# DuckTapeDevOps/kubernetes-cloud

Measured on AMD Instinct MI355X. Metric: GPT-J-6B finetune tokens/sec, higher is better.
Workload: dtype bf16; 1 GPU; model=gpt-j-6b, global_batch=32, micro_batch=16, grad_accum=2, seq_len=2048, parallelism=dp1, activation_checkpointing=False

## Files before the change

csrc/kernels/attention.hip:

```cpp
#include "common.h"

#define LOG2E 1.4426950408889634f
#define LN2 0.6931471805599453f

struct AttnParams {
  const bf16_t* q; const bf16_t* k; const bf16_t* v;
  bf16_t* o; float* lse;
  long long q_sb, q_st, q_sh, k_sb, k_st, k_sh, v_sb, v_st, v_sh;
  long long o_sb, o_st, o_sh;
  int B, Sq, Sk, H, Hkv, d_real, causal;
  float scale;
  const float* alibi;
  const int* kv_len;
  const int* fix_flags;
  int window;
  const unsigned* key_mask;
  int km_words;
};

struct AttnBwdParams {
  const bf16_t* q; const bf16_t* k; const bf16_t* v; const bf16_t* o;
  const bf16_t* dout; bf16_t* dq; bf16_t* dk; bf16_t* dv;
  const float* lse; const float* delta;
  long long q_sb, q_st, q_sh, k_sb, k_st, k_sh, v_sb, v_st, v_sh;
// ... 886 lines not shown
    if (causal) {
      hipLaunchKernelGGL((attn_bwd_dkdv_kernel<256, true>), g1w, dim3(256), 0, stream, p);
      hipLaunchKernelGGL((attn_bwd_dq32_kernel<256, true>), h2, dim3(256), 0, stream, p);
    } else {
      hipLaunchKernelGGL((attn_bwd_dkdv_kernel<256, false>), g1w, dim3(256), 0, stream, p);
      hipLaunchKernelGGL((attn_bwd_dq32_kernel<256, false>), h2, dim3(256), 0, stream, p);
    }
    return 0;
  }
  dim3 g1(((Sk + 63) / 64) * B * Hkv);
  dim3 g2(((Sq + 63) / 64) * B * H);
  ATTN_D_DISPATCH(D, {
    if (causal) {
      hipLaunchKernelGGL((attn_bwd_dkdv_kernel<DD, true>), g1, dim3(256), 0, stream, p);
      hipLaunchKernelGGL((attn_bwd_dq_kernel<DD, true>), g2, dim3(256), 0, stream, p);
    } else {
      hipLaunchKernelGGL((attn_bwd_dkdv_kernel<DD, false>), g1, dim3(256), 0, stream, p);
      hipLaunchKernelGGL((attn_bwd_dq_kernel<DD, false>), g2, dim3(256), 0, stream, p);
    }
  });
  return 0;
}

KCA_API int kca_attn_bwd(const void* q, const void* k, const void* v,
                         const void* o, const void* dout, void* dq, void* dk,
                         void* dv, const float* lse, const float* delta,
                         long long q_sb, long long q_st, long long q_sh,
                         long long k_sb, long long k_st, long long k_sh,
                         long long v_sb, long long v_st, long long v_sh,
                         long long do_sb, long long do_st, long long do_sh,
                         long long dq_sb, long long dq_st, long long dq_sh,
                         long long dk_sb, long long dk_st, long long dk_sh,
                         long long dv_sb, long long dv_st, long long dv_sh,
                         int B, int Sq, int Sk, int H, int Hkv, int d_real,
                         int causal, float scale, const float* alibi,
                         const int* kv_len, int window, const unsigned* key_mask, hipStream_t stream) {
  return kca_attn_bwd_ws(q, k, v, o, dout, dq, dk, dv, lse, delta, q_sb, q_st, q_sh, k_sb, k_st, k_sh, v_sb, v_st,
                         v_sh, do_sb, do_st, do_sh, dq_sb, dq_st, dq_sh, dk_sb, dk_st, dk_sh, dv_sb, dv_st, dv_sh,
                         B, Sq, Sk, H, Hkv, d_real, causal, scale, alibi, kv_len, window, key_mask, nullptr, 0,
                         stream);
}
```

csrc/kernels/attention_tiled.hip:

```cpp
#include "common.h"

#include <type_traits>

namespace {

constexpr float kLog2e = 1.4426950408889634f;
constexpr float kLn2 = 0.6931471805599453f;
constexpr float kRescaleThr = 8.0f;

#ifdef KCA_ATTN_STAMPS
__device__ unsigned long long g_attn_stamps[64];
__device__ __forceinline__ unsigned long long ast_now() {
  unsigned long long t;
  __builtin_amdgcn_sched_barrier(0);
  asm volatile("s_memtime %0\n\ts_waitcnt lgkmcnt(0)" : "=s"(t)::"memory");
  __builtin_amdgcn_sched_barrier(0);
  return t;
}
#define ASTAMP_DECL                                            \
  unsigned long long st_acc_[8] = {0, 0, 0, 0, 0, 0, 0, 0}; \
  unsigned long long st_prev_ = ast_now();
#define ASTAMP(k)                           \
  do {                                      \
    const unsigned long long n_ = ast_now(); \
// ... 206 lines not shown
  constexpr int NCH = D / 8, RB = D * 2, NCS = DS / 8;
  const int l32 = lane & 31, hh = lane >> 5;
#pragma unroll
  for (int db = 0; db < D / 32; ++db) {
#pragma unroll
    for (int g = 0; g < 4; ++g) {
      uint2 w;
      w.x = pk_bf16(acc[db][4 * g] * mul, acc[db][4 * g + 1] * mul);
      w.y = pk_bf16(acc[db][4 * g + 2] * mul, acc[db][4 * g + 3] * mul);
      *reinterpret_cast<uint2*>(lds + l32 * RB + ((4 * db + g + l32) % NCH) * 16 + hh * 8) = w;
    }
  }
  asm volatile("" ::: "memory");
  static_assert((32 * NCS) % 64 == 0, "whole-wave epilogue rounds");
#pragma unroll
  for (int j = 0; j < 32 * NCS / 64; ++j) {
    const int idx = j * 64 + lane, r = idx / NCS, c = idx % NCS;
    const uint4 v = *reinterpret_cast<const uint4*>(lds + r * RB + ((c + r) % NCH) * 16);
    *reinterpret_cast<uint4*>(row0 + (long long)r * st + c * 8) = v;
  }
  asm volatile("" ::: "memory");
}

template <int D, bool CAUSAL, int OC = -1, int DS = D, int MC = -1>
__global__ void __launch_bounds__(256, (D <= 128 ? 2 : 1)) attn_fwd_tiled_kernel(FastFwdParams p) {
  constexpr int BM = 128, BN = 32;
  constexpr int TILE = BN * D * 2;
  constexpr int KS = DS / 16;
  using Stg = StagerFor<D, DS>;
  constexpr int CPT = Stg::CPT;
  __shared__ __attribute__((aligned(16))) char smem[3 * 2 * TILE];

  ASTAMP_DECL
  const int tid = threadIdx.x, lane = tid & 63, wave = tid >> 6;
  const int l32 = lane & 31, hh = lane >> 5, gi = lane & 15;
  const int nqb = p.Sq / BM;
  const int lid = xcd_remap(blockIdx.x, gridDim.x);
  const int qi = lid % nqb;
  const int qb = CAUSAL ? (nqb - 1 - qi) : qi;
  const int bh = lid / nqb;
  const int b = bh / p.H, h = bh % p.H;
  const int hk = h / (p.H / p.Hkv);
  const int off = p.Sk - p.Sq;
  const int q0 = qb * BM + wave * 32;
  const int qrow = q0 + l32;
  int kv_hi = p.Sk;
// ... 420 lines not shown
  const float inv = ltot > 0.f ? 1.f / ltot : 0.f;
  if (hh == 0 && p.lse)
    p.lse[((long long)b * p.H + h) * p.Sq + qrow] = ltot > 0.f ? (m + log2f(ltot)) * kLn2 : INFINITY;
  asm volatile("s_waitcnt vmcnt(0) lgkmcnt(0)" ::: "memory");
  __syncthreads();
  store_tile_lds<D, D>(p.o + b * p.o_sb + h * p.o_sh + (long long)q0 * p.o_st, p.o_st, oacc, lane, inv,
                       smem + wave * 32 * D * 2);
  ASTAMP(6);
  ASTAMP_FLUSH(48);
}

struct FastBwdParams {
  const bf16_t* q; const bf16_t* k; const bf16_t* v; const bf16_t* dout;
  bf16_t* dq; bf16_t* dk; bf16_t* dv;
  const float* lse; const float* delta;
  long long q_sb, q_st, q_sh, k_sb, k_st, k_sh, v_sb, v_st, v_sh, do_sb, do_st, do_sh;
  long long dq_sb, dq_st, dq_sh, dk_sb, dk_st, dk_sh, dv_sb, dv_st, dv_sh;
  int B, Sq, Sk, H, Hkv;
  float scale;
};
struct FastBwdWsParams : FastBwdParams {
  bf16_t* ws;
};

template <int D>
__device__ __forceinline__ void row_bases(int l32, int hh, int& e, int& o) {
  const int xr = (l32 >> 2) & 3;
  e = (l32 >> 3) * 16 * D + 64 * (l32 & 7) + 16 * (hh ^ xr);
  o = (l32 >> 3) * 16 * D + 64 * (l32 & 7) + 16 * ((2 + hh) ^ xr);
}
template <int D>
__device__ __forceinline__ void tr_bases(int lane, int& b1, int& b2) {
  const int hh = lane >> 5, gi = lane & 15;
  const int c3 = 2 * ((lane >> 4) & 1) + ((gi & 3) >> 1);
  b1 = 64 * (4 * hh + (gi >> 2)) + 16 * (c3 ^ hh) + 8 * (gi & 1);
  b2 = 16 * D + 64 * (4 * hh + (gi >> 2)) + 16 * (c3 ^ hh ^ 2) + 8 * (gi & 1);
}
template <int D>
__device__ __forceinline__ bf16x8 tr_frag(const char* img, int b1, int b2, int s, int db) {
  return cat8(lds_tr4(img, b1 + 2 * s * 16 * D + 512 * db), lds_tr4(img, b2 + 2 * s * 16 * D + 512 * db));
}
template <int D>
__device__ __forceinline__ bf16x8 row_frag(const char* img, int be, int bo, int s) {
  return lds_b128(img, ((s & 1) ? bo : be) + 512 * (s >> 1));
}

// ... 132 lines not shown
          t1[(db + 1) & 1] = tr_frag<D>(Ks, b1, b2, 1, db + 1);
          __builtin_amdgcn_sched_group_barrier(0x100, 4, 0);
        }
        dq[db] = __builtin_amdgcn_mfma_f32_32x32x16_bf16(t0[db & 1], d0, dq[db], 0, 0, 0);
        dq[db] = __builtin_amdgcn_mfma_f32_32x32x16_bf16(t1[db & 1], d1, dq[db], 0, 0, 0);
        __builtin_amdgcn_sched_group_barrier(0x8, 2, 0);
      }
    }
    ASTAMP(4);
    asm volatile("" ::: "memory");
    if (t + 1 < ntiles) stg.store(sk, sv, smem + ((t + 1) & 1) * 2 * TILE);
    __syncthreads();
    ASTAMP(5);
  };
  const int nfree = CAUSAL ? ntiles - 4 : ntiles;
  for (int t = 0; t < nfree; ++t) tile_step(t, std::false_type{});
  for (int t = max(nfree, 0); t < ntiles; ++t) tile_step(t, std::true_type{});
  store_tile_lds<D, DS>(p.dq + b * p.dq_sb + h * p.dq_sh + (long long)q0 * p.dq_st, p.dq_st, dq, lane, p.scale,
                        smem + wave * 32 * D * 2);
  ASTAMP(6);
  ASTAMP_FLUSH(16);
}

template <int D, bool CAUSAL>
__global__ void __launch_bounds__(256, 2) attn_bwd_dq_ds_kernel(FastBwdWsParams p) {
  constexpr int BM = 128, BN = 32;
  constexpr int TILE = BN * D * 2;
  constexpr int NCH = D / 8, CPT = 32 * NCH / 256, RPI = 256 / NCH;
  constexpr int DST = BN * 32 * 2;
  constexpr int DOFF = 2 * TILE;
  __shared__ __attribute__((aligned(16))) char smem[4 * TILE];
  static_assert(DOFF + 2 * 4 * DST <= 4 * TILE && 256 % NCH == 0, "dQ from dS: LDS plan");

  const int tid = threadIdx.x, lane = tid & 63, wave = tid >> 6;
  const int hh = lane >> 5;
  const int nqb = p.Sq / BM;
  const int lid = xcd_remap(blockIdx.x, gridDim.x);
  const int qi = lid % nqb;
  const int qb = CAUSAL ? (nqb - 1 - qi) : qi;
  const int bh = lid / nqb;
  const int b = bh / p.H, h = bh % p.H;
  const int off = p.Sk - p.Sq;
  const int q0 = qb * BM + wave * 32;
  int kv_hi = p.Sk;
  if (CAUSAL) kv_hi = min(kv_hi, qb * BM + BM + off);
  const int ntiles = (kv_hi + BN - 1) / BN;

  f32x16 dq[D / 32];
// ... 73 lines not shown
      t0[0] = tr_frag<D>(Ks, b1, b2, 0, 0);
      t1[0] = tr_frag<D>(Ks, b1, b2, 1, 0);
      __builtin_amdgcn_sched_group_barrier(0x100, 8, 0);
#pragma unroll
      for (int db = 0; db < D / 32; ++db) {
        if (db + 1 < D / 32) {
          t0[(db + 1) & 1] = tr_frag<D>(Ks, b1, b2, 0, db + 1);
          t1[(db + 1) & 1] = tr_frag<D>(Ks, b1, b2, 1, db + 1);
          __builtin_amdgcn_sched_group_barrier(0x100, 4, 0);
        }
        dq[db] = __builtin_amdgcn_mfma_f32_32x32x16_bf16(t0[db & 1], d0, dq[db], 0, 0, 0);
        dq[db] = __builtin_amdgcn_mfma_f32_32x32x16_bf16(t1[db & 1], d1, dq[db], 0, 0, 0);
        __builtin_amdgcn_sched_group_barrier(0x8, 2, 0);
      }
    }
    asm volatile("" ::: "memory");
    if (t + 1 < ntiles) store_tile((t + 1) & 1, std::integral_constant<int, NX>{});
    load_k(min(t + 2, last));
    load_ds(min(t + 1 + PD, last), std::integral_constant<int, NX>{});
    __syncthreads();
  };
  for (int t = 0; t < ntiles; t += PD)
    static_for<0, PD>([&](auto J) { tile_step(t + decltype(J)::value, J); });
  store_tile_lds<D>(p.dq + b * p.dq_sb + h * p.dq_sh + (long long)q0 * p.dq_st, p.dq_st, dq, lane, p.scale,
                    smem + wave * 32 * D * 2);
}

template <int D, bool CAUSAL, int DS = D>
__global__ void __launch_bounds__(256, (D <= 64 && !CAUSAL) ? 3 : 1) attn_bwd_dkdv_tiled_kernel(FastBwdParams p) {
  constexpr int BK = 128, BQ = 32;
  constexpr int TILE = BQ * D * 2;
  using Stg = StagerFor<D, DS>;
  constexpr int NCH = D / 8, NCS = DS / 8, CPT = Stg::CPT;
  constexpr int KSD = DS / 16;
  constexpr int VOFF = 4 * TILE;
  constexpr int LOFF = VOFF + 4 * TILE;
  __shared__ __attribute__((aligned(16))) char smem[LOFF + 2 * 64 * 4];
  ASTAMP_DECL

  const int tid = threadIdx.x, lane = tid & 63, wave = tid >> 6;
  const int l32 = lane & 31, hh = lane >> 5;
  const int nkb = p.Sk / BK;
  const int lid = xcd_remap(blockIdx.x, gridDim.x);
  const int kb = lid % nkb, bh = lid / nkb;
  const int b = bh / p.Hkv, hk = bh % p.Hkv;
  const int grp = p.H / p.Hkv;
  const int off = p.Sk - p.Sq;
  const int kw = kb * BK + wave * 32;
// ... 171 lines not shown

template <bool ON>
struct DsEmitter {
  __device__ __forceinline__ void init(const FastBwdParams&, int, int, int, int) {}
  __device__ __forceinline__ void store(const bf16x8&, const bf16x8&, int) const {}
};
template <>
struct DsEmitter<true> {
  __amdgpu_buffer_rsrc_t r_;
  int v_, dt_, t0_;
  __device__ __forceinline__ void init(const FastBwdWsParams& p, int bh, int lane, int q_lo, int kw) {
    r_ = head_rsrc(p.ws + (long long)bh * p.Sq * p.Sk);
    v_ = lane * 16;
    dt_ = (p.Sk / 32) * 2048;
    t0_ = (q_lo / 32) * dt_ + (kw / 32) * 2048;
  }
  __device__ __forceinline__ void store(const bf16x8& s0, const bf16x8& s1, int t) const {
    const int so = __builtin_amdgcn_readfirstlane(t0_ + t * dt_);
    __builtin_amdgcn_raw_buffer_store_b128(*reinterpret_cast<const u32x4*>(&s0), r_, v_, so, 2);
    __builtin_amdgcn_raw_buffer_store_b128(*reinterpret_cast<const u32x4*>(&s1), r_, v_, so + 1024, 2);
  }
};

template <int D, bool CAUSAL, bool EMIT_DS = false>
__global__ void __launch_bounds__(512, 1)
    attn_bwd_dkdv_w8_kernel(std::conditional_t<EMIT_DS, FastBwdWsParams, FastBwdParams> p) {
  constexpr int BK = 128, BQ = 32;
  constexpr int TILE = BQ * D * 2;
  using Stg = Stager<D, true, 512>;
  constexpr int CPT = Stg::CPT, KSD = D / 16;
  constexpr int PSZ = 4 * 64 * 16;
  constexpr int POFF = 3 * 2 * TILE;
  constexpr int LOFF = POFF + 2 * 4 * PSZ;
  __shared__ __attribute__((aligned(16))) char smem[LOFF + 3 * 64 * 4];
  static_assert(8 * 32 * D * 2 <= LOFF, "epilogue images of the 8 waves");
  ASTAMP_DECL

  const int tid = threadIdx.x, lane = tid & 63;
  const int wave = __builtin_amdgcn_readfirstlane(tid >> 6);
  const int pw = wave & 3;
  const bool kside = wave < 4;
  const int l32 = lane & 31, hh = lane >> 5;
  const int nkb = p.Sk / BK;
  const int lid = xcd_remap(blockIdx.x, gridDim.x);
  const int kb = lid % nkb, bh = lid / nkb;
  const int b = bh / p.H, h = bh % p.H;
  const int off = p.Sk - p.Sq;
  const int kw = kb * BK + pw * 32;
  const int key = kw + l32;
// ... 187 lines not shown
      }
      ASTAMP(4);
      asm volatile("" ::: "memory");
      if (t + 2 < total) store_tile(nxt);
      __syncthreads();
      ASTAMP(5);
    };
    if (total > 1) {
      load_tile(1);
      store_tile(1);
    }
    __syncthreads();
    int cur = 0;
    for (int t = 0; t < total; ++t) {
      const int nxt = cur == 0 ? 2 : cur - 1;
      k_step(t, cur, nxt);
      cur = cur == 2 ? 0 : cur + 1;
    }
  }
  __builtin_amdgcn_s_setprio(0);
  {
    bf16_t* dst = kside ? p.dk + b * p.dk_sb + h * p.dk_sh + (long long)kw * p.dk_st
                        : p.dv + b * p.dv_sb + h * p.dv_sh + (long long)kw * p.dv_st;
    store_tile_lds<D>(dst, kside ? p.dk_st : p.dv_st, acc, lane, kside ? p.scale : 1.f, smem + wave * 32 * D * 2);
  }
  ASTAMP(6);
  if (!kside) {
    ASTAMP_FLUSH(40);
  } else {
    ASTAMP_FLUSH(56);
  }
}

inline bool offsets_fit(long long rows, long long stride) { return (rows + 128) * stride * 2 < (1ll << 31); }

}

static int g_attn_variant = 7;
KCA_API int kca_attn_set_variant(int v) {
  g_attn_variant = v;
  return 0;
}

KCA_API int kca_attn_fwd_tiled(const void* q, const void* k, const void* v, void* o, float* lse,
                               long long q_sb, long long q_st, long long q_sh, long long k_sb,
                               long long k_st, long long k_sh, long long v_sb, long long v_st,
                               long long v_sh, long long o_sb, long long o_st, long long o_sh,
                               int B, int Sq, int Sk, int H, int Hkv, int d, int causal,
                               float scale, int rowsum_col, int max_col, int* flags, hipStream_t stream) {
  if ((d != 48 && d != 64 && d != 96 && d != 128 && d != 160 && d != 256) || Sq % 128 || Sk % 32 || Sq <= 0 ||
      H % Hkv || !flags)
    return 1;
  if (max_col >= 0 && (max_col != 40 || rowsum_col != 40 || d != 48)) return 1;
  if (d == 48 && causal) return 1;
  if (rowsum_col >= 0 && (rowsum_col != 40 || (d != 64 && d != 48) || causal)) return 1;
  if (causal && Sk < Sq) return 1;
  if (!offsets_fit(Sk, k_st) || !offsets_fit(Sk, v_st)) return 1;
  FastFwdParams p{(const bf16_t*)q, (const bf16_t*)k, (const bf16_t*)v, (bf16_t*)o, lse, flags,
                  q_sb, q_st, q_sh, k_sb, k_st, k_sh, v_sb, v_st, v_sh, o_sb, o_st, o_sh,
                  B, Sq, Sk, H, Hkv, scale};
  dim3 grid((Sq / 128) * B * H);
// ... 131 lines not shown
  const long long need = kca_attn_bwd_ws_bytes(B, Sq, Sk, H, Hkv, d, causal);
  if ((g_attn_variant & 6) != 6 || !ws || need == 0 || ws_bytes < need || !offsets_fit(Sk, k_st) ||
      !offsets_fit(Sk, v_st) || !offsets_fit(Sq, q_st) || !offsets_fit(Sq, do_st))
    return kca_attn_bwd_tiled(q, k, v, dout, dq, dk, dv, lse, delta, q_sb, q_st, q_sh, k_sb, k_st, k_sh, v_sb,
                              v_st, v_sh, do_sb, do_st, do_sh, dq_sb, dq_st, dq_sh, dk_sb, dk_st, dk_sh, dv_sb,
                              dv_st, dv_sh, B, Sq, Sk, H, Hkv, d, causal, scale, stream);
  FastBwdWsParams p{{(const bf16_t*)q, (const bf16_t*)k, (const bf16_t*)v, (const bf16_t*)dout,
                     (bf16_t*)dq, (bf16_t*)dk, (bf16_t*)dv, lse, delta,
                     q_sb, q_st, q_sh, k_sb, k_st, k_sh, v_sb, v_st, v_sh, do_sb, do_st, do_sh,
                     dq_sb, dq_st, dq_sh, dk_sb, dk_st, dk_sh, dv_sb, dv_st, dv_sh,
                     B, Sq, Sk, H, Hkv, scale},
                    (bf16_t*)ws};
  dim3 g1((Sk / 128) * B * H), g2((Sq / 128) * B * H);
  if (causal) {
    hipLaunchKernelGGL((attn_bwd_dkdv_w8_kernel<256, true, true>), g1, dim3(512), 0, stream, p);
    hipLaunchKernelGGL((attn_bwd_dq_ds_kernel<256, true>), g2, dim3(256), 0, stream, p);
  } else {
    hipLaunchKernelGGL((attn_bwd_dkdv_w8_kernel<256, false, true>), g1, dim3(512), 0, stream, p);
    hipLaunchKernelGGL((attn_bwd_dq_ds_kernel<256, false>), g2, dim3(256), 0, stream, p);
  }
  return 0;
}

#ifdef KCA_ATTN_STAMPS
KCA_API int kca_attn_stamps(unsigned long long* host, int reset) {
  if (hipMemcpyFromSymbol(host, HIP_SYMBOL(g_attn_stamps), sizeof(unsigned long long) * 64) != hipSuccess) return 1;
  if (reset) {
    unsigned long long z[64] = {0};
    if (hipMemcpyToSymbol(HIP_SYMBOL(g_attn_stamps), z, sizeof(z)) != hipSuccess) return 1;
  }
  return 0;
}
#endif
```

csrc/kernels/common.h:

```cpp
#pragma once
#include <hip/hip_runtime.h>
#include <hip/hip_bf16.h>
#include <stdint.h>

#define KCA_API extern "C" __attribute__((visibility("default")))

typedef uint16_t bf16_t;
typedef float f32x4 __attribute__((ext_vector_type(4)));
typedef float f32x16 __attribute__((ext_vector_type(16)));
typedef short s16x8 __attribute__((ext_vector_type(8)));
typedef short s16x4 __attribute__((ext_vector_type(4)));
typedef __bf16 bf16x8 __attribute__((ext_vector_type(8)));
typedef __bf16 bf16x4 __attribute__((ext_vector_type(4)));

#ifdef KCA_DEBUG
#define KCA_DASSERT(cond)                                                                                  \
  do {                                                                                                     \
    if (!(cond)) {                                                                                         \
      printf("KCA_DASSERT failed %s:%d: %s (block %d,%d,%d thread %d)\n", __FILE__, __LINE__, #cond,         \
             (int)blockIdx.x, (int)blockIdx.y, (int)blockIdx.z, (int)threadIdx.x);                         \
      __builtin_trap();                                                                                    \
    }                                                                                                      \
  } while (0)
#else
// ... 7 lines not shown
  return __uint_as_float(((uint32_t)b) << 16);
}

__device__ __forceinline__ uint16_t f2bf(float f) {
  __bf16 h = (__bf16)f;
  return __builtin_bit_cast(uint16_t, h);
}

__device__ __forceinline__ uint32_t pack_bf16x2(float lo, float hi) {
  return (uint32_t)f2bf(lo) | ((uint32_t)f2bf(hi) << 16);
}

__device__ __forceinline__ void load8(const bf16_t* p, float (&x)[8]) {
  U16x8 u = *reinterpret_cast<const U16x8*>(p);
#pragma unroll
  for (int i = 0; i < 8; ++i) x[i] = bf2f(u.v[i]);
}

__device__ __forceinline__ void store8(bf16_t* p, const float (&x)[8]) {
  U16x8 u;
#pragma unroll
  for (int i = 0; i < 8; ++i) u.v[i] = f2bf(x[i]);
  *reinterpret_cast<U16x8*>(p) = u;
}

__device__ __forceinline__ void load8f(const float* p, float (&x)[8]) {
  float4 a = *reinterpret_cast<const float4*>(p);
  float4 b = *reinterpret_cast<const float4*>(p + 4);
  x[0] = a.x; x[1] = a.y; x[2] = a.z; x[3] = a.w;
  x[4] = b.x; x[5] = b.y; x[6] = b.z; x[7] = b.w;
}

__device__ __forceinline__ void store8f(float* p, const float (&x)[8]) {
  *reinterpret_cast<float4*>(p) = make_float4(x[0], x[1], x[2], x[3]);
  *reinterpret_cast<float4*>(p + 4) = make_float4(x[4], x[5], x[6], x[7]);
}

template <int DT>
__device__ __forceinline__ float e2f(uint32_t u16) {
  if constexpr (DT == 0) return __uint_as_float(u16 << 16);
  else return (float)__builtin_bit_cast(_Float16, (uint16_t)u16);
}
template <int DT>
__device__ __forceinline__ uint32_t f2e(float f) {
  if constexpr (DT == 0) return (uint32_t)f2bf(f);
  else return (uint32_t)__builtin_bit_cast(uint16_t, (_Float16)f);
// ... 110 lines not shown
```

csrc/kernels/elementwise.hip:

```cpp
#include "common.h"

__device__ __forceinline__ float gelu_erf(float x) {
  return 0.5f * x * (1.f + erff(x * 0.7071067811865476f));
}
__device__ __forceinline__ float gelu_erf_grad(float x) {
  const float cdf = 0.5f * (1.f + erff(x * 0.7071067811865476f));
  const float pdf = 0.3989422804014327f * __expf(-0.5f * x * x);
  return cdf + x * pdf;
}

template <bool TANH, int DT = 0>
__global__ void gelu_fwd_kernel(const bf16_t* __restrict__ u,
                                bf16_t* __restrict__ y, long long n8) {
  for (long long i = blockIdx.x * (long long)blockDim.x + threadIdx.x; i < n8;
       i += (long long)gridDim.x * blockDim.x) {
    float v[8];
    load8_t<DT>(u + i * 8, v);
#pragma unroll
    for (int j = 0; j < 8; ++j) v[j] = TANH ? gelu_tanh(v[j]) : gelu_erf(v[j]);
    store8_t<DT>(y + i * 8, v);
  }
}

template <bool TANH>
// ... 100 lines not shown
                            const float* __restrict__ sin_t,
                            const int* __restrict__ pos_ids, float sign) {
  const int half = rot >> 1;
  const int groups = half >> 2;
  const int nh = nh_q + nh_k;
  const long long total = tokens * nh * groups;
  for (long long idx = blockIdx.x * (long long)blockDim.x + threadIdx.x;
       idx < total; idx += (long long)gridDim.x * blockDim.x) {
    const int g = idx % groups;
    const long long th = idx / groups;
    const int hh = th % nh;
    const long long t = th / nh;
    const int pos = pos_ids ? pos_ids[t] : (int)(t % seq);
    bf16_t* base = hh < nh_q ? q + t * tok_stride_q + hh * head_stride_q
                             : k + t * tok_stride_k + (hh - nh_q) * head_stride_k;
    const float* ct = cos_t + (size_t)pos * half + g * 4;
    const float* st = sin_t + (size_t)pos * half + g * 4;
    float c[4], s[4];
#pragma unroll
    for (int j = 0; j < 4; ++j) { c[j] = ct[j]; s[j] = sign * st[j]; }
    if (interleaved) {
      float x[8];
      load8(base + g * 8, x);
#pragma unroll
      for (int j = 0; j < 4; ++j) {
        float a = x[2 * j], b = x[2 * j + 1];
        x[2 * j] = a * c[j] - b * s[j];
        x[2 * j + 1] = b * c[j] + a * s[j];
      }
      store8(base + g * 8, x);
    } else {
      U16x4 ua = *reinterpret_cast<const U16x4*>(base + g * 4);
      U16x4 ub = *reinterpret_cast<const U16x4*>(base + half + g * 4);
      U16x4 oa, ob;
#pragma unroll
      for (int j = 0; j < 4; ++j) {
        float a = bf2f(ua.v[j]), b = bf2f(ub.v[j]);
        oa.v[j] = f2bf(a * c[j] - b * s[j]);
        ob.v[j] = f2bf(b * c[j] + a * s[j]);
      }
      *reinterpret_cast<U16x4*>(base + g * 4) = oa;
      *reinterpret_cast<U16x4*>(base + half + g * 4) = ob;
    }
  }
}

__global__ void rope_scalar_kernel(bf16_t* __restrict__ q,
                                   bf16_t* __restrict__ k, int nh_q, int nh_k,
                                   long long tokens, int seq,
                                   long long tok_stride_q,
                                   long long head_stride_q,
                                   long long tok_stride_k,
// ... 375 lines not shown
```

kubernetes_cloud_amd/ops/_lib.py:

```python
from __future__ import annotations

import ctypes
import os
import threading

import torch

_HERE = os.path.dirname(os.path.abspath(__file__))
LIB_DIR = os.path.join(os.path.dirname(_HERE), "_lib")
DEBUG = os.environ.get("KCA_DEBUG", "0") in ("1", "true")
KERNEL_LIB = os.path.join(LIB_DIR, "libkca_kernels_debug.so" if DEBUG else "libkca_kernels.so")
KERNEL_LIB = os.environ.get("KCA_KERNEL_LIB") or KERNEL_LIB
ATTN_VARIANT_ENV = os.environ.get("KCA_ATTN_VARIANT")

_lock = threading.Lock()
_lib = None
_err: str | None = None

P = ctypes.c_void_p
I = ctypes.c_int
LL = ctypes.c_longlong
F = ctypes.c_float

_SIGS = {
# ... 8 lines not shown
    "kca_quick_gelu_fwd": [P, P, LL, P],
    "kca_quick_gelu_bwd": [P, P, P, LL, P],
    "kca_geglu_fwd": [P, P, LL, I, P],
    "kca_add_bias_nhwc": [P, P, P, P, LL, I, P],
    "kca_add_bias2_nhwc": [P, P, P, P, P, LL, I, P],
    "kca_colsum_bf16": [P, P, I, I, I, P],
    "kca_geglu_bwd": [P, P, P, LL, I, P],
    "kca_rope": [P, P, I, I, LL, I, LL, LL, LL, LL, I, I, P, P, P, F, P],
    "kca_accum_grad": [P, P, F, I, LL, P],
    "kca_accum_grad_pair": [P, P, P, F, LL, P],
    "kca_accum_grad_multi": [P, I, F, P],
    "kca_cast_f32_bf16": [P, P, LL, P],
    "kca_ema": [P, P, F, LL, P],
    "kca_cross_entropy_fwd": [P, LL, P, I, I, I, P, P, P],
    "kca_cross_entropy_bwd": [P, LL, P, P, P, F, I, I, I, P, LL, P],
    "kca_adamw": [P, P, P, P, P, LL, P, F, F, F, F, F, F, F, P, P, P],
    "kca_sumsq": [P, LL, P, P, P],
    "kca_adamw8bit": [P, P, P, P, P, P, P, LL, P, F, F, F, F, F, F, F, P, P, P],
    "kca_clip_coef": [P, F, F, P, P, P, P],
    "kca_attn_fwd": [P] * 5 + [LL] * 12 + [I] * 7 + [F, P, P, I, P, I, I, P, P],
    "kca_attn_bwd_preprocess": [P, P, P, LL, LL, LL, LL, LL, LL, I, I, I, I, P],
    "kca_attn_bwd": [P] * 10 + [LL] * 21 + [I] * 7 + [F, P, P, I, P, P],
    "kca_attn_bwd_ws": [P] * 10 + [LL] * 21 + [I] * 7 + [F, P, P, I, P, P, LL, P],
    "kca_attn_bwd_ws_bytes": [I] * 7,
    "kca_attn_fwd_wide": [P] * 5 + [LL] * 12 + [I] * 6 + [F, P, P],
    "kca_attn_set_tiled": [I],
    "kca_attn_set_variant": [I],
    "kca_transpose_bf16": [P, LL, P, LL, I, I, P],
    "kca_gelu_fwd_t": [P, LL, P, LL, P, LL, I, I, I, P],
    "kca_gelu_bwd_t": [P, LL, P, LL, P, LL, P, LL, P, I, I, I, P],
    "kca_transpose_colsum": [P, LL, P, LL, P, I, I, P],
    "kca_col_reduce_f32": [P, I, I, P, P, P],
    "kca_accum_grad_2d": [P, P, LL, I, I, F, I, P],
    "kca_groupnorm_fwd": [P, P, P, P, P, P, P, I, I, I, I, F, I, P],
    "kca_groupnorm_bwd": [P, P, P, P, P, P, P, P, P, P, I, I, I, I, I, P],
    "kca_groupnorm_nhwc_ws": [I, I, I],
    "kca_groupnorm_nhwc_fwd": [P, P, P, P, P, P, P, I, I, I, I, F, I, P],
    "kca_groupnorm_nhwc_fwd_add": [P, P, P, P, LL, P, P, P, P, I, I, I, I, F, I, P],
    "kca_groupnorm_nhwc_cat_fwd": [P, P, P, P, P, P, P, P, P, P, I, I, I, I, I, I, F, I, P],
    "kca_groupnorm_nhwc_bwd": [P, P, P, P, P, P, P, P, P, P, I, I, I, I, I, P],
    "kca_skinny_set_smallk": [I],
    "kca_conv3x3_fwd": [P, P, P, P, I, I, I, I, I, P],
    "kca_conv3x3_set_variant": [I],
    "kca_conv3x3_wflip": [P, P, I, I, P],
    "kca_conv3x3_wgrad_splits": [I, I, I, I, I],
    "kca_conv3x3_wgrad": [P, P, P, P, I, I, I, I, I, I, P],
# ... 137 lines not shown
```

kubernetes_cloud_amd/ops/attention.py:

```python
from __future__ import annotations

import math

import torch

from . import _lib
from .rope import apply_rotary_


def attention_reference(q, k, v, causal: bool, scale: float | None = None,
                        kv_len: torch.Tensor | None = None, alibi: torch.Tensor | None = None,
                        window: int = 0):
    B, Sq, H, D = q.shape
    Sk, Hkv = k.shape[1], k.shape[2]
    scale = scale if scale is not None else 1.0 / math.sqrt(D)
    qf = q.float().transpose(1, 2)
    kf = k.float().transpose(1, 2)
    vf = v.float().transpose(1, 2)
    if Hkv != H:
        rep = H // Hkv
        kf = kf.repeat_interleave(rep, dim=1)
        vf = vf.repeat_interleave(rep, dim=1)
    s = torch.matmul(qf, kf.transpose(-1, -2)) * scale
    qi = torch.arange(Sq, device=q.device)[:, None]
    ki = torch.arange(Sk, device=q.device)[None, :]
    off = Sk - Sq
    if alibi is not None:
        s = s + alibi.float().view(1, H, 1, 1) * (ki - qi - off).float()
    mask = torch.zeros(B, 1, Sq, Sk, dtype=torch.bool, device=q.device)
    if causal:
        mask = mask | (ki > qi + off)
    if window:
        mask = mask | (ki <= qi + off - window)
    if kv_len is not None and kv_len.dtype == torch.bool:
        mask = mask | ~kv_len.to(q.device).view(B, 1, 1, Sk)
    elif kv_len is not None:
        mask = mask | (ki[None, None] >= kv_len.view(B, 1, 1, 1).to(q.device))
    s = s.masked_fill(mask, float("-inf"))
    lse = torch.logsumexp(s, dim=-1)
    p = torch.exp(s - lse[..., None])
    p = torch.nan_to_num(p, nan=0.0)
    o = torch.matmul(p, vf).transpose(1, 2)
    return o.to(q.dtype), lse


def set_tiled_path(enable: bool) -> None:
    _lib.call("kca_attn_set_tiled", int(bool(enable)))


DEFAULT_VARIANT = 7
_VARIANT = [int(_lib.ATTN_VARIANT_ENV) if _lib.ATTN_VARIANT_ENV is not None else DEFAULT_VARIANT]


def set_variant(v: int) -> int:
    _lib.call("kca_attn_set_variant", int(v))
    old, _VARIANT[0] = _VARIANT[0], int(v)
    return old


def _strides(t):
    return t.stride(0), t.stride(1), t.stride(2)


def pack_key_mask(mask: torch.Tensor) -> torch.Tensor:
    B, Sk = mask.shape
    W = (Sk + 31) // 32
    m = torch.zeros(B, W * 32, dtype=torch.int64, device=mask.device)
    m[:, :Sk] = mask.to(torch.int64)
    words = (m.view(B, W, 32) << torch.arange(32, device=mask.device, dtype=torch.int64)).sum(-1)
    words = torch.where(words >= 2 ** 31, words - 2 ** 32, words)
    return words.to(torch.int32).contiguous()


# ... 8 lines not shown
    B, Sq, H, D = q.shape
    Sk, Hkv = k.shape[1], k.shape[2]
    o = out if out is not None else torch.empty(B, Sq, H, D, device=q.device, dtype=q.dtype)
    if lse is None:
        lse = torch.empty(B, H, Sq, device=q.device, dtype=torch.float32)
    if flags is None:
        flags = torch.empty(4 * ((Sq + 127) // 128) * B * H, device=q.device, dtype=torch.int32)
    lens, km = _masks(kv_len)
    _lib.call("kca_attn_fwd", q.data_ptr(), k.data_ptr(), v.data_ptr(), o.data_ptr(), lse.data_ptr(),
              *_strides(q), *_strides(k), *_strides(v), *_strides(o),
              B, Sq, Sk, H, Hkv, D, int(causal), float(scale), _lib.ptr(alibi), _lib.ptr(lens),
              int(window), _lib.ptr(km), int(rowsum_col), int(max_col), flags.data_ptr(), _lib.stream())
    return o, lse


def bwd_workspace(q, k, causal):
    if not _VARIANT[0] & 4:
        return None
    B, Sq, H, D = q.shape
    n = _lib.require().kca_attn_bwd_ws_bytes(B, Sq, k.shape[1], H, k.shape[2], D, int(causal))
    return torch.empty(n, device=q.device, dtype=torch.uint8) if n > 0 else None


def _bwd(q, k, v, o, do, lse, dq, dk, dv, causal, scale, kv_len, alibi, window: int = 0, ws=None):
    B, Sq, H, D = q.shape
    Sk, Hkv = k.shape[1], k.shape[2]
    delta = torch.empty(B, H, Sq, device=q.device, dtype=torch.float32)
    _lib.call("kca_attn_bwd_preprocess", o.data_ptr(), do.data_ptr(), delta.data_ptr(),
              *_strides(o), *_strides(do), B, Sq, H, D, _lib.stream())
    args = (q.data_ptr(), k.data_ptr(), v.data_ptr(), o.data_ptr(), do.data_ptr(),
            dq.data_ptr(), dk.data_ptr(), dv.data_ptr(), lse.data_ptr(), delta.data_ptr(),
            *_strides(q), *_strides(k), *_strides(v), *_strides(do),
            *_strides(dq), *_strides(dk), *_strides(dv),
            B, Sq, Sk, H, Hkv, D, int(causal), float(scale), _lib.ptr(alibi), _lib.ptr(_masks(kv_len)[0]),
            int(window), _lib.ptr(_masks(kv_len)[1]))
    if ws is None:
        _lib.call("kca_attn_bwd", *args, _lib.stream())
    else:
        _lib.call("kca_attn_bwd_ws", *args, ws.data_ptr(), ws.numel() * ws.element_size(), _lib.stream())


def _check(q, k, v):
    for t in (q, k, v):
        if t.dim() != 4 or t.stride(-1) != 1:
            raise ValueError("attention expects [B, S, H, D] views with unit last stride")
        if t.dtype != torch.bfloat16:
            raise ValueError("native attention is bf16")
    D = q.shape[-1]
    if D % 8 or D > 256:
        raise ValueError(f"head_dim {D} unsupported (multiple of 8, <= 256)")


class _FlashAttnFn(torch.autograd.Function):
    @staticmethod
    def forward(ctx, q, k, v, causal, scale, kv_len, alibi, window):
        _check(q, k, v)
        o, lse = _fwd(q, k, v, causal, scale, kv_len, alibi, window=window)
        ctx.save_for_backward(q, k, v, o, lse, kv_len, alibi)
        ctx.causal, ctx.scale, ctx.window = causal, scale, window
        return o

    @staticmethod
# ... 116 lines not shown
```

kubernetes_cloud_amd/ops/fused_block.py:

```python
from __future__ import annotations

import torch
import torch.nn.functional as F

from . import _lib, grad_sink
from .attention import _bwd as _attn_bwd
from .attention import _fwd as _attn_fwd
from .attention import bwd_workspace as _attn_bwd_workspace
from .attention import native_mask
from .linear import transpose
from .rope import apply_rotary_


def eligible(cfg) -> bool:
    d, f = cfg.hidden, cfg.ffn_dim
    return (cfg.parallel_residual and cfg.shared_ln and cfg.rotary_dim > 0 and not cfg.qkv_bias
            and not cfg.out_bias and not cfg.alibi and not cfg.attention_layers
            and d % 64 == 0 and f % 64 == 0 and cfg.head_dim in (64, 128, 256))


class FusedParallelBlock:

    def __init__(self, blk):
        self.blk = blk
        self.tanh = blk.mlp.approx == "tanh"

    def refresh(self):
        pass

# ... 73 lines not shown
        dev, dt = x.device, x.dtype
        st = _lib.stream()
        dm2 = dm.reshape(T, d).contiguous() if dm is not None else torch.zeros(T, d, device=dev, dtype=dt)
        da2 = da.reshape(T, d).contiguous() if da is not None else torch.zeros(T, d, device=dev, dtype=dt)

        dmt = torch.empty(d, T, device=dev, dtype=dt)
        part = torch.empty(T // 64, d, device=dev, dtype=torch.float32) if b_needed(mlp.fc_out) else None
        _lib.call("kca_transpose_colsum", dm2.data_ptr(), d, dmt.data_ptr(), T, _lib.ptr(part), T, d, st)
        g_b_out = _emit(mlp.fc_out.bias, _col_sums(part, dt)) if part is not None else None
        dg = F.linear(dm2, mlp.fc_out.weight_t)
        g_fc_out = _emit_wgrad(mlp.fc_out.weight, dmt, gt)
        if da2.data_ptr() != dm2.data_ptr():
            dat = transpose(da2)
        else:
            dat = dmt
        g_out = _emit_wgrad(a.out.weight, dat, transpose(o))
        do = F.linear(da2, a.out.weight_t).view(B, S, H, D)
        del dat, dmt

        q5 = qkv.view(B, S, 3, H, D)
        dqkv = torch.empty_like(qkv)
        d5 = dqkv.view(B, S, 3, H, D)
        dq, dk, dv = d5[:, :, 0], d5[:, :, 1], d5[:, :, 2]
        _attn_bwd(q5[:, :, 0], q5[:, :, 1], q5[:, :, 2], o.view(B, S, H, D), do, lse, dq, dk, dv, True,
                  a.scale, kv_len, None, ws=_attn_bwd_workspace(q5[:, :, 0], q5[:, :, 1], True))
        apply_rotary_(dq, dk, cfg.rotary_dim, S, cfg.rotary_interleaved, cfg.rotary_base, -1.0)
        del do

        du = torch.empty_like(u)
        dut = torch.empty(f, T, device=dev, dtype=dt)
        part = torch.empty(T // 64, f, device=dev, dtype=torch.float32) if b_needed(mlp.fc_in) else None
        _lib.call("kca_gelu_bwd_t", dg.data_ptr(), f, u.data_ptr(), f, du.data_ptr(), f, dut.data_ptr(), T,
                  _lib.ptr(part), T, f, int(fb.tanh), st)
        del dg
        g_b_in = _emit(mlp.fc_in.bias, _col_sums(part, dt)) if part is not None else None

        dx = None
        if ctx.needs_input_grad[0]:
            dx = F.linear(dqkv, a.qkv.weight_t)
            dx.addmm_(du, mlp.fc_in.weight_t.t())
        xt = transpose(x.reshape(T, d))
        g_fc_in = _emit_wgrad(mlp.fc_in.weight, dut, xt)
        del dut, du
        g_qkv = _emit_wgrad(a.qkv.weight, transpose(dqkv), xt)
        return (dx.view(B, S, d) if dx is not None else None, g_qkv, g_out, g_fc_in, g_b_in, g_fc_out, g_b_out,
                None, None)


def b_needed(lin) -> bool:
    return lin.bias is not None and lin.bias.requires_grad


__all__ = ["FusedParallelBlock", "eligible"]
```

Measured before the change: 35190 tokens/s.

## Fuse inverse RoPE and dQKV transpose into attention backward epilogues

Adds a transposing epilogue to the tiled attention backward kernels (dkdv and dq). It applies the inverse rotary rotation to dQ/dK in LDS and writes both the row-major dqkv and a transposed dqkv_t used directly by the QKV weight-gradient GEMM. This removes the separate apply_rotary_ pass and the standalone transpose of dqkv. In exchange it adds a block-wide sync and extra strided global writes in the epilogue, and it makes variant 15 the default.

```diff
diff --git a/csrc/kernels/attention.hip b/csrc/kernels/attention.hip
--- a/csrc/kernels/attention.hip
+++ b/csrc/kernels/attention.hip
@@ -932,6 +932,41 @@
   return 0;
 }
 
+KCA_API int kca_attn_bwd_tiled_t(const void* q, const void* k, const void* v, const void* dout,
+                                 void* dq, void* dk, void* dv, const float* lse, const float* delta,
+                                 long long q_sb, long long q_st, long long q_sh, long long k_sb,
+                                 long long k_st, long long k_sh, long long v_sb, long long v_st,
+                                 long long v_sh, long long do_sb, long long do_st, long long do_sh,
+                                 long long dq_sb, long long dq_st, long long dq_sh, long long dk_sb,
+                                 long long dk_st, long long dk_sh, long long dv_sb, long long dv_st,
+                                 long long dv_sh, int B, int Sq, int Sk, int H, int Hkv, int d,
+                                 int causal, float scale, void* ws, long long ws_bytes, void* dT, long long ldT,
+                                 const float* cos_t, const float* sin_t, int rot, int interleaved, int seq,
+                                 hipStream_t stream);
+
+KCA_API int kca_attn_bwd_ws_t(const void* q, const void* k, const void* v,
+                              const void* o, const void* dout, void* dq, void* dk,
+                              void* dv, const float* lse, const float* delta,
+                              long long q_sb, long long q_st, long long q_sh,
+                              long long k_sb, long long k_st, long long k_sh,
+                              long long v_sb, long long v_st, long long v_sh,
+                              long long do_sb, long long do_st, long long do_sh,
+                              long long dq_sb, long long dq_st, long long dq_sh,
+                              long long dk_sb, long long dk_st, long long dk_sh,
+                              long long dv_sb, long long dv_st, long long dv_sh,
+                              int B, int Sq, int Sk, int H, int Hkv, int d_real,
+                              int causal, float scale, const float* alibi,
+                              const int* kv_len, int window, const unsigned* key_mask, void* ws,
+                              long long ws_bytes, void* dqkvT, long long ldT, const float* cos_t,
+                              const float* sin_t, int rot, int interleaved, int seq, hipStream_t stream) {
+  (void)o;
+  if (d_real % 8 || H % Hkv || window || !g_attn_tiled || alibi || kv_len || key_mask) return 2;
+  return kca_attn_bwd_tiled_t(q, k, v, dout, dq, dk, dv, lse, delta, q_sb, q_st, q_sh, k_sb, k_st, k_sh, v_sb,
+                              v_st, v_sh, do_sb, do_st, do_sh, dq_sb, dq_st, dq_sh, dk_sb, dk_st, dk_sh, dv_sb,
+                              dv_st, dv_sh, B, Sq, Sk, H, Hkv, d_real, causal, scale, ws, ws_bytes, dqkvT, ldT,
+                              cos_t, sin_t, rot, interleaved, seq, stream);
+}
+
 KCA_API int kca_attn_bwd(const void* q, const void* k, const void* v,
                          const void* o, const void* dout, void* dq, void* dk,
                          void* dv, const float* lse, const float* delta,
diff --git a/csrc/kernels/attention_tiled.hip b/csrc/kernels/attention_tiled.hip
--- a/csrc/kernels/attention_tiled.hip
+++ b/csrc/kernels/attention_tiled.hip
@@ -252,6 +252,80 @@
   asm volatile("" ::: "memory");
 }
 
+__device__ __forceinline__ unsigned perm_lo16(unsigned a, unsigned b) {
+  return __builtin_amdgcn_perm(b, a, 0x05040100u);
+}
+__device__ __forceinline__ unsigned perm_hi16(unsigned a, unsigned b) {
+  return __builtin_amdgcn_perm(b, a, 0x07060302u);
+}
+template <int D>
+__device__ __forceinline__ void store_tile_lds_t(bf16_t* row0, long long st, const f32x16 (&acc)[D / 32], int lane,
+                                                 float mul, char* grp, int wsub, bf16_t* trow0, long long ldT,
+                                                 const float* cos_t, const float* sin_t, int rot, int pos0,
+                                                 float rsign) {
+  constexpr int NCH = D / 8, RB = D * 2, IMG = 32 * RB;
+  static_assert(D == 256, "transposing epilogue: four waves x 64 dims");
+  asm volatile("" : "+v"(lane));
+  char* lds = grp + wsub * IMG;
+  const int l32 = lane & 31, hh = lane >> 5;
+#pragma unroll
+  for (int db = 0; db < D / 32; ++db) {
+#pragma unroll
+    for (int g = 0; g < 4; ++g) {
+      uint2 w;
+      w.x = pk_bf16(acc[db][4 * g] * mul, acc[db][4 * g + 1] * mul);
+      w.y = pk_bf16(acc[db][4 * g + 2] * mul, acc[db][4 * g + 3] * mul);
+      *reinterpret_cast<uint2*>(lds + l32 * RB + ((4 * db + g + l32) % NCH) * 16 + hh * 8) = w;
+    }
+  }
+  asm volatile("" ::: "memory");
+  if (rot > 0) {
+    const int half = rot >> 1;
+    const float* ct = cos_t + (size_t)(pos0 + l32) * half;
+    const float* sn = sin_t + (size_t)(pos0 + l32) * half;
+    for (int ch = hh; ch < (rot >> 3); ch += 2) {
+      bf16_t* a = reinterpret_cast<bf16_t*>(lds + l32 * RB + ((ch + l32) % NCH) * 16);
+      const float4 c4 = *reinterpret_cast<const float4*>(ct + ch * 4);
+      const float4 s4 = *reinterpret_cast<const float4*>(sn + ch * 4);
+      const float c[4] = {c4.x, c4.y, c4.z, c4.w};
+      const float s[4] = {rsign * s4.x, rsign * s4.y, rsign * s4.z, rsign * s4.w};
+      float x[8];
+      load8(a, x);
+      rope_rotate8_interleaved(x, c, s);
+      store8(a, x);
+    }
+    asm volatile("" ::: "memory");
+  }
+#pragma unroll
+  for (int j = 0; j < 32 * NCH / 64; ++j) {
+    const int idx = j * 64 + lane, r = idx / NCH, c = idx % NCH;
+    const uint4 v = *reinterpret_cast<const uint4*>(lds + r * RB + ((c + r) % NCH) * 16);
+    *reinterpret_cast<uint4*>(row0 + (long long)r * st + c * 8) = v;
+  }
+  __syncthreads();
+  const int tg = lane & 15, dc = lane >> 4, rb = (tg & 3) * 8;
+  const char* src = grp + (tg >> 2) * IMG + rb * RB;
+  bf16_t* tp = trow0 + tg * 8;
+#pragma unroll
+  for (int rd = 0; rd < 2; ++rd) {
+    const int c = 8 * wsub + 4 * rd + dc;
+    u32x4 a[8];
+#pragma unroll
+    for (int i = 0; i < 8; ++i) a[i] = *reinterpret_cast<const u32x4*>(src + i * RB + ((c + rb + i) % NCH) * 16);
+#pragma unroll
+    for (int j = 0; j < 8; ++j) {
+      u32x4 bj;
+#pragma unroll
+      for (int k = 0; k < 4; ++k) {
+        const unsigned x = a[2 * k][j >> 1], y = a[2 * k + 1][j >> 1];
+        bj[k] = (j & 1) ? perm_hi16(x, y) : perm_lo16(x, y);
+      }
+      *reinterpret_cast<u32x4*>(tp + (long long)(8 * c + j) * ldT) = bj;
+    }
+  }
+  asm volatile("" ::: "memory");
+}
+
 template <int D, bool CAUSAL, int OC = -1, int DS = D, int MC = -1>
 __global__ void __launch_bounds__(256, (D <= 128 ? 2 : 1)) attn_fwd_tiled_kernel(FastFwdParams p) {
   constexpr int BM = 128, BN = 32;
@@ -718,6 +792,14 @@
 struct FastBwdWsParams : FastBwdParams {
   bf16_t* ws;
 };
+struct FastBwdTParams : FastBwdWsParams {
+  bf16_t* dT;
+  long long ldT;
+  const float* cos_t;
+  const float* sin_t;
+  int rot;
+  float rsign;
+};
 
 template <int D>
 __device__ __forceinline__ void row_bases(int l32, int hh, int& e, int& o) {
@@ -896,8 +978,9 @@
   ASTAMP_FLUSH(16);
 }
 
-template <int D, bool CAUSAL>
-__global__ void __launch_bounds__(256, 2) attn_bwd_dq_ds_kernel(FastBwdWsParams p) {
+template <int D, bool CAUSAL, bool EMIT_T = false>
+__global__ void __launch_bounds__(256, 2)
+    attn_bwd_dq_ds_kernel(std::conditional_t<EMIT_T, FastBwdTParams, FastBwdWsParams> p) {
   constexpr int BM = 128, BN = 32;
   constexpr int TILE = BN * D * 2;
   constexpr int NCH = D / 8, CPT = 32 * NCH / 256, RPI = 256 / NCH;
@@ -1017,8 +1100,14 @@
   };
   for (int t = 0; t < ntiles; t += PD)
     static_for<0, PD>([&](auto J) { tile_step(t + decltype(J)::value, J); });
-  store_tile_lds<D>(p.dq + b * p.dq_sb + h * p.dq_sh + (long long)q0 * p.dq_st, p.dq_st, dq, lane, p.scale,
-                    smem + wave * 32 * D * 2);
+  bf16_t* const dst = p.dq + b * p.dq_sb + h * p.dq_sh + (long long)q0 * p.dq_st;
+  if constexpr (EMIT_T) {
+    store_tile_lds_t<D>(dst, p.dq_st, dq, lane, p.scale, smem, __builtin_amdgcn_readfirstlane(wave),
+                        p.dT + (long long)h * D * p.ldT + (long long)b * p.Sq + qb * BM, p.ldT, p.cos_t, p.sin_t,
+                        p.rot, q0, p.rsign);
+  } else {
+    store_tile_lds<D>(dst, p.dq_st, dq, lane, p.scale, smem + wave * 32 * D * 2);
+  }
 }
 
 template <int D, bool CAUSAL, int DS = D>
@@ -1236,9 +1325,11 @@
   }
 };
 
-template <int D, bool CAUSAL, bool EMIT_DS = false>
+template <int D, bool CAUSAL, bool EMIT_DS = false, bool EMIT_T = false>
 __global__ void __launch_bounds__(512, 1)
-    attn_bwd_dkdv_w8_kernel(std::conditional_t<EMIT_DS, FastBwdWsParams, FastBwdParams> p) {
+    attn_bwd_dkdv_w8_kernel(std::conditional_t<EMIT_T, FastBwdTParams,
+                                               std::conditional_t<EMIT_DS, FastBwdWsParams, FastBwdParams>> p) {
+  static_assert(EMIT_DS || !EMIT_T, "the transposing epilogue comes with the dS workspace");
   constexpr int BK = 128, BQ = 32;
   constexpr int TILE = BQ * D * 2;
   using Stg = Stager<D, true, 512>;
@@ -1472,7 +1563,15 @@
   {
     bf16_t* dst = kside ? p.dk + b * p.dk_sb + h * p.dk_sh + (long long)kw * p.dk_st
                         : p.dv + b * p.dv_sb + h * p.dv_sh + (long long)kw * p.dv_st;
-    store_tile_lds<D>(dst, kside ? p.dk_st : p.dv_st, acc, lane, kside ? p.scale : 1.f, smem + wave * 32 * D * 2);
+    if constexpr (EMIT_T) {
+      const int which = kside ? 1 : 2;
+      store_tile_lds_t<D>(dst, kside ? p.dk_st : p.dv_st, acc, lane, kside ? p.scale : 1.f,
+                          smem + (kside ? 0 : 4) * 32 * D * 2, pw,
+                          p.dT + (long long)(which * p.H + h) * D * p.ldT + (long long)b * p.Sk + kb * BK, p.ldT,
+                          p.cos_t, p.sin_t, kside ? p.rot : 0, kw, p.rsign);
+    } else {
+      store_tile_lds<D>(dst, kside ? p.dk_st : p.dv_st, acc, lane, kside ? p.scale : 1.f, smem + wave * 32 * D * 2);
+    }
   }
   ASTAMP(6);
   if (!kside) {
@@ -1486,7 +1585,7 @@
 
 }
 
-static int g_attn_variant = 7;
+static int g_attn_variant = 15;
 KCA_API int kca_attn_set_variant(int v) {
   g_attn_variant = v;
   return 0;
@@ -1664,6 +1763,52 @@
   return 0;
 }
 
+KCA_API int kca_attn_bwd_tiled_t(const void* q, const void* k, const void* v, const void* dout,
+                                 void* dq, void* dk, void* dv, const float* lse, const float* delta,
+                                 long long q_sb, long long q_st, long long q_sh, long long k_sb,
+                                 long long k_st, long long k_sh, long long v_sb, long long v_st,
+                                 long long v_sh, long long do_sb, long long do_st, long long do_sh,
+                                 long long dq_sb, long long dq_st, long long dq_sh, long long dk_sb,
+                                 long long dk_st, long long dk_sh, long long dv_sb, long long dv_st,
+                                 long long dv_sh, int B, int Sq, int Sk, int H, int Hkv, int d,
+                                 int causal, float scale, void* ws, long long ws_bytes, void* dT, long long ldT,
+                                 const float* cos_t, const float* sin_t, int rot, int interleaved, int seq,
+                                 hipStream_t stream) {
+  const long long need = kca_attn_bwd_ws_bytes(B, Sq, Sk, H, Hkv, d, causal);
+  if ((g_attn_variant & 14) != 14 || !ws || need == 0 || ws_bytes < need || !offsets_fit(Sk, k_st) ||
+      !offsets_fit(Sk, v_st) || !offsets_fit(Sq, q_st) || !offsets_fit(Sq, do_st))
+    return 2;
+  if (Sq != Sk || !dq || !dT) return 2;
+  const long long hd = (long long)H * d, T = (long long)B * Sq;
+  const bf16_t* const d0 = (const bf16_t*)dq;
+  if ((const bf16_t*)dk != d0 + hd || (const bf16_t*)dv != d0 + 2 * hd) return 2;
+  if (dq_sh != d || dk_sh != d || dv_sh != d || dq_st != 3 * hd || dk_st != 3 * hd || dv_st != 3 * hd ||
+      dq_sb != Sq * 3 * hd || dk_sb != dq_sb || dv_sb != dq_sb)
+    return 2;
+  if (ldT < T || ldT % 8 || (long long)d * ldT * 2 >= (1ll << 31)) return 2;
+  if ((reinterpret_cast<uintptr_t>(dq) | reinterpret_cast<uintptr_t>(dT)) & 15) return 2;
+  if (rot < 0 || rot > d || rot % 8) return 2;
+  if (rot > 0 && (!interleaved || !cos_t || !sin_t || seq != Sq ||
+                  ((reinterpret_cast<uintptr_t>(cos_t) | reinterpret_cast<uintptr_t>(sin_t)) & 15)))
+    return 2;
+  FastBwdTParams p{{{(const bf16_t*)q, (const bf16_t*)k, (const bf16_t*)v, (const bf16_t*)dout,
+                     (bf16_t*)dq, (bf16_t*)dk, (bf16_t*)dv, lse, delta,
+                     q_sb, q_st, q_sh, k_sb, k_st, k_sh, v_sb, v_st, v_sh, do_sb, do_st, do_sh,
+                     dq_sb, dq_st, dq_sh, dk_sb, dk_st, dk_sh, dv_sb, dv_st, dv_sh,
+                     B, Sq, Sk, H, Hkv, scale},
+                    (bf16_t*)ws},
+                   (bf16_t*)dT, ldT, cos_t, sin_t, rot, -1.f};
+  dim3 g1((Sk / 128) * B * H), g2((Sq / 128) * B * H);
+  if (causal) {
+    hipLaunchKernelGGL((attn_bwd_dkdv_w8_kernel<256, true, true, true>), g1, dim3(512), 0, stream, p);
+    hipLaunchKernelGGL((attn_bwd_dq_ds_kernel<256, true, true>), g2, dim3(256), 0, stream, p);
+  } else {
+    hipLaunchKernelGGL((attn_bwd_dkdv_w8_kernel<256, false, true, true>), g1, dim3(512), 0, stream, p);
+    hipLaunchKernelGGL((attn_bwd_dq_ds_kernel<256, false, true>), g2, dim3(256), 0, stream, p);
+  }
+  return 0;
+}
+
 #ifdef KCA_ATTN_STAMPS
 KCA_API int kca_attn_stamps(unsigned long long* host, int reset) {
   if (hipMemcpyFromSymbol(host, HIP_SYMBOL(g_attn_stamps), sizeof(unsigned long long) * 64) != hipSuccess) return 1;
diff --git a/csrc/kernels/common.h b/csrc/kernels/common.h
--- a/csrc/kernels/common.h
+++ b/csrc/kernels/common.h
@@ -53,6 +53,15 @@
 #pragma unroll
   for (int i = 0; i < 8; ++i) u.v[i] = f2bf(x[i]);
   *reinterpret_cast<U16x8*>(p) = u;
+}
+
+__device__ __forceinline__ void rope_rotate8_interleaved(float (&x)[8], const float (&c)[4], const float (&s)[4]) {
+#pragma unroll
+  for (int j = 0; j < 4; ++j) {
+    float a = x[2 * j], b = x[2 * j + 1];
+    x[2 * j] = a * c[j] - b * s[j];
+    x[2 * j + 1] = b * c[j] + a * s[j];
+  }
 }
 
 __device__ __forceinline__ void load8f(const float* p, float (&x)[8]) {
diff --git a/csrc/kernels/elementwise.hip b/csrc/kernels/elementwise.hip
--- a/csrc/kernels/elementwise.hip
+++ b/csrc/kernels/elementwise.hip
@@ -146,12 +146,7 @@
     if (interleaved) {
       float x[8];
       load8(base + g * 8, x);
-#pragma unroll
-      for (int j = 0; j < 4; ++j) {
-        float a = x[2 * j], b = x[2 * j + 1];
-        x[2 * j] = a * c[j] - b * s[j];
-        x[2 * j + 1] = b * c[j] + a * s[j];
-      }
+      rope_rotate8_interleaved(x, c, s);
       store8(base + g * 8, x);
     } else {
       U16x4 ua = *reinterpret_cast<const U16x4*>(base + g * 4);
diff --git a/kubernetes_cloud_amd/ops/_lib.py b/kubernetes_cloud_amd/ops/_lib.py
--- a/kubernetes_cloud_amd/ops/_lib.py
+++ b/kubernetes_cloud_amd/ops/_lib.py
@@ -54,6 +54,7 @@
     "kca_attn_bwd_preprocess": [P, P, P, LL, LL, LL, LL, LL, LL, I, I, I, I, P],
     "kca_attn_bwd": [P] * 10 + [LL] * 21 + [I] * 7 + [F, P, P, I, P, P],
     "kca_attn_bwd_ws": [P] * 10 + [LL] * 21 + [I] * 7 + [F, P, P, I, P, P, LL, P],
+    "kca_attn_bwd_ws_t": [P] * 10 + [LL] * 21 + [I] * 7 + [F, P, P, I, P, P, LL, P, LL, P, P, I, I, I, P],
     "kca_attn_bwd_ws_bytes": [I] * 7,
     "kca_attn_fwd_wide": [P] * 5 + [LL] * 12 + [I] * 6 + [F, P, P],
     "kca_attn_set_tiled": [I],
diff --git a/kubernetes_cloud_amd/ops/attention.py b/kubernetes_cloud_amd/ops/attention.py
--- a/kubernetes_cloud_amd/ops/attention.py
+++ b/kubernetes_cloud_amd/ops/attention.py
@@ -5,7 +5,7 @@
 import torch
 
 from . import _lib
-from .rope import apply_rotary_
+from .rope import apply_rotary_, rope_tables
 
 
 def attention_reference(q, k, v, causal: bool, scale: float | None = None,
@@ -48,7 +48,7 @@
     _lib.call("kca_attn_set_tiled", int(bool(enable)))
 
 
-DEFAULT_VARIANT = 7
+DEFAULT_VARIANT = 15
 _VARIANT = [int(_lib.ATTN_VARIANT_ENV) if _lib.ATTN_VARIANT_ENV is not None else DEFAULT_VARIANT]
 
 
@@ -103,22 +103,58 @@
     return torch.empty(n, device=q.device, dtype=torch.uint8) if n > 0 else None
 
 
-def _bwd(q, k, v, o, do, lse, dq, dk, dv, causal, scale, kv_len, alibi, window: int = 0, ws=None):
-    B, Sq, H, D = q.shape
-    Sk, Hkv = k.shape[1], k.shape[2]
-    delta = torch.empty(B, H, Sq, device=q.device, dtype=torch.float32)
+def _delta(o, do):
+    B, Sq, H, D = o.shape
+    delta = torch.empty(B, H, Sq, device=o.device, dtype=torch.float32)
     _lib.call("kca_attn_bwd_preprocess", o.data_ptr(), do.data_ptr(), delta.data_ptr(),
               *_strides(o), *_strides(do), B, Sq, H, D, _lib.stream())
-    args = (q.data_ptr(), k.data_ptr(), v.data_ptr(), o.data_ptr(), do.data_ptr(),
+    return delta
+
+
+def _bwd_args(q, k, v, o, do, lse, delta, dq, dk, dv, causal, scale, kv_len=None, alibi=None, window: int = 0):
+    B, Sq, H, D = q.shape
+    Sk, Hkv = k.shape[1], k.shape[2]
+    return (q.data_ptr(), k.data_ptr(), v.data_ptr(), o.data_ptr(), do.data_ptr(),
             dq.data_ptr(), dk.data_ptr(), dv.data_ptr(), lse.data_ptr(), delta.data_ptr(),
             *_strides(q), *_strides(k), *_strides(v), *_strides(do),
             *_strides(dq), *_strides(dk), *_strides(dv),
             B, Sq, Sk, H, Hkv, D, int(causal), float(scale), _lib.ptr(alibi), _lib.ptr(_masks(kv_len)[0]),
             int(window), _lib.ptr(_masks(kv_len)[1]))
+
+
+def _bwd(q, k, v, o, do, lse, dq, dk, dv, causal, scale, kv_len, alibi, window: int = 0, ws=None, delta=None):
+    if delta is None:
+        delta = _delta(o, do)
+    args = _bwd_args(q, k, v, o, do, lse, delta, dq, dk, dv, causal, scale, kv_len, alibi, window)
     if ws is None:
         _lib.call("kca_attn_bwd", *args, _lib.stream())
     else:
         _lib.call("kca_attn_bwd_ws", *args, ws.data_ptr(), ws.numel() * ws.element_size(), _lib.stream())
+
+
+def bwd_t_enabled() -> bool:
+    return bool(_VARIANT[0] & 8)
+
+
+def _bwd_t(q, k, v, o, do, lse, dqkv, dqkv_t, causal, scale, rot, interleaved, base, ws) -> bool:
+    B, S, three, H, D = dqkv.shape
+    dq, dk, dv = dqkv[:, :, 0], dqkv[:, :, 1], dqkv[:, :, 2]
+    if (ws is None or not _VARIANT[0] & 8 or three != 3 or not dqkv.is_contiguous() or not (0 <= rot <= D)
+            or rot % 8 or (rot > 0 and not interleaved)):
+        _bwd(q, k, v, o, do, lse, dq, dk, dv, causal, scale, None, None, ws=ws)
+        return False
+    cos = sin = None
+    if rot > 0:
+        cos, sin = rope_tables(rot, max(S, 1), base, q.device)
+    delta = _delta(o, do)
+    rc = _lib.call_rc("kca_attn_bwd_ws_t", *_bwd_args(q, k, v, o, do, lse, delta, dq, dk, dv, causal, scale),
+                      ws.data_ptr(), ws.numel() * ws.element_size(), dqkv_t.data_ptr(), dqkv_t.stride(0),
+                      _lib.ptr(cos), _lib.ptr(sin), int(rot), int(bool(interleaved)), S, _lib.stream())
+    if rc == 2:
+        _bwd(q, k, v, o, do, lse, dq, dk, dv, causal, scale, None, None, ws=ws, delta=delta)
+    elif rc != 0:
+        raise RuntimeError(f"kca_attn_bwd_ws_t returned status {rc}")
+    return rc == 0
 
 
 def _check(q, k, v):
diff --git a/kubernetes_cloud_amd/ops/fused_block.py b/kubernetes_cloud_amd/ops/fused_block.py
--- a/kubernetes_cloud_amd/ops/fused_block.py
+++ b/kubernetes_cloud_amd/ops/fused_block.py
@@ -5,6 +5,8 @@
 
 from . import _lib, grad_sink
 from .attention import _bwd as _attn_bwd
+from .attention import _bwd_t as _attn_bwd_t
+from .attention import bwd_t_enabled as _attn_bwd_t_on
 from .attention import _fwd as _attn_fwd
 from .attention import bwd_workspace as _attn_bwd_workspace
 from .attention import native_mask
@@ -124,10 +126,19 @@
         dqkv = torch.empty_like(qkv)
         d5 = dqkv.view(B, S, 3, H, D)
         dq, dk, dv = d5[:, :, 0], d5[:, :, 1], d5[:, :, 2]
-        _attn_bwd(q5[:, :, 0], q5[:, :, 1], q5[:, :, 2], o.view(B, S, H, D), do, lse, dq, dk, dv, True,
-                  a.scale, kv_len, None, ws=_attn_bwd_workspace(q5[:, :, 0], q5[:, :, 1], True))
-        apply_rotary_(dq, dk, cfg.rotary_dim, S, cfg.rotary_interleaved, cfg.rotary_base, -1.0)
-        del do
+        ws = _attn_bwd_workspace(q5[:, :, 0], q5[:, :, 1], True)
+        dqkv_t = None
+        if _attn_bwd_t_on() and kv_len is None and ws is not None and a.qkv.weight.requires_grad:
+            dqkv_t = torch.empty(3 * d, T, device=dev, dtype=dt)
+            if not _attn_bwd_t(q5[:, :, 0], q5[:, :, 1], q5[:, :, 2], o.view(B, S, H, D), do, lse, d5, dqkv_t,
+                               True, a.scale, cfg.rotary_dim, cfg.rotary_interleaved, cfg.rotary_base, ws):
+                dqkv_t = None
+        else:
+            _attn_bwd(q5[:, :, 0], q5[:, :, 1], q5[:, :, 2], o.view(B, S, H, D), do, lse, dq, dk, dv, True,
+                      a.scale, kv_len, None, ws=ws)
+        if dqkv_t is None:
+            apply_rotary_(dq, dk, cfg.rotary_dim, S, cfg.rotary_interleaved, cfg.rotary_base, -1.0)
+        del do, ws
 
         du = torch.empty_like(u)
         dut = torch.empty(f, T, device=dev, dtype=dt)
@@ -144,7 +155,7 @@
         xt = transpose(x.reshape(T, d))
         g_fc_in = _emit_wgrad(mlp.fc_in.weight, dut, xt)
         del dut, du
-        g_qkv = _emit_wgrad(a.qkv.weight, transpose(dqkv), xt)
+        g_qkv = _emit_wgrad(a.qkv.weight, dqkv_t if dqkv_t is not None else transpose(dqkv), xt)
         return (dx.view(B, S, d) if dx is not None else None, g_qkv, g_out, g_fc_in, g_b_in, g_fc_out, g_b_out,
                 None, None)
 
```

Measured after the change: 35420 tokens/s (median of 6 runs). Within noise of the previous version (+0.7%).
